# cts198859/deeprl_signal_control

Measured on AMD Instinct MI355X. Metric: env-steps/s (agents x envs x sim-steps/s), large_grid MA2C, higher is better.
Workload: dtype f32; 1 GPU; large_grid 5x5 (25 agents), MA2C LSTM policy (neighbour fingerprint gather), 1024 env instances per GPU; step = 120 control steps (x5 sim-steps) of every instance + 1 A2C update (BPTT, clip, RMSProp); envs_per_gpu=1024, n_step=120, agents=25, parallelism=env-sharded x1, live_vehicles=window mean over the timed region

## Files before the change

deeprl_signal_control_amd/_lib.py:

```python
import ctypes as C
import os

import numpy as np

HERE = os.path.dirname(os.path.abspath(__file__))
LIB_PATH = os.environ.get('TSC_LIB') or os.path.join(HERE, 'libtsc.so')

_fp = C.POINTER(C.c_float)
_ip = C.POINTER(C.c_int32)
_bp = C.POINTER(C.c_uint8)


class TscScenario(C.Structure):
    _fields_ = [
        ('n_lane', C.c_int32), ('n_route', C.c_int32), ('n_agent', C.c_int32), ('n_flow', C.c_int32),
        ('k_max', C.c_int32), ('p_max', C.c_int32), ('l_max', C.c_int32), ('s_max', C.c_int32),
        ('nbr_max', C.c_int32),
        ('lane_len', _fp), ('lane_vmax', _fp), ('lane_det_start', _fp),
        ('lane_node', _ip), ('lane_up', _ip),
        ('mv_next', _ip), ('mv_link', _ip), ('mv_yield', _ip), ('mv_prio', _ip), ('mv_zip', _ip), ('route_entry', _ip), ('flows', _ip),
        ('agent_lanes', _ip), ('agent_nlane', _ip), ('agent_nlink', _ip), ('agent_nphase', _ip),
        ('green_tab', _bp), ('yellow_tab', _bp),
        ('nbr', _ip), ('obs_kind', _ip), ('obs_src', _ip),
        ('control_interval_sec', C.c_int32), ('yellow_interval_sec', C.c_int32),
        ('episode_length_sec', C.c_int32), ('teleport_sec', C.c_int32),
        ('queue_cap', C.c_int32), ('objective', C.c_int32), ('agent_kind', C.c_int32),
        ('realnet_scale', C.c_int32),
        ('coop_gamma', C.c_double), ('norm_wave', C.c_double), ('norm_wait', C.c_double),
        ('clip_wave', C.c_double), ('clip_wait', C.c_double), ('coef_wait', C.c_double),
        ('lane_origin', _fp),
        ('n_stream', C.c_int32), ('k_choice', C.c_int32),
        ('stream_entry', _ip), ('stream_origin', _fp), ('stream_limit', _fp), ('stream_mode', _ip), ('stream_choice', _ip),
        ('n_interval', C.c_int32), ('choice_interval_sec', C.c_int32),
        ('lane_sib', _ip),
    ]


_LIB = None

SYMBOLS = ['tsc_last_error', 'tsc_version', 'tsc_profile_enable', 'tsc_profile_select', 'tsc_profile_reset', 'tsc_profile_read',
           'tsc_profile_name', 'tsc_env_create', 'tsc_env_destroy', 'tsc_env_set_stream', 'tsc_env_set_resident_instances',
           'tsc_env_reset', 'tsc_env_set_stream_routes', 'tsc_env_set_demand', 'tsc_env_demand', 'tsc_env_set_greedy', 'tsc_env_greedy_actions', 'tsc_env_set_pressure', 'tsc_env_pressure_actions', 'tsc_env_set_actuated', 'tsc_env_actuated_actions', 'tsc_env_actuated_state', 'tsc_env_set_reward_pressure', 'tsc_env_fixed_time_actions', 'tsc_env_set_fingerprint', 'tsc_env_bind_fingerprint', 'tsc_env_reward_sum', 'tsc_env_step', 'tsc_env_step_plan', 'tsc_env_get_state',
           'tsc_env_live_vehicles', 'tsc_env_vehicle_counts', 'tsc_env_set_block_order', 'tsc_env_counters', 'tsc_env_debug_clock', 'tsc_env_live_sum', 'tsc_env_record', 'tsc_env_read_record', 'tsc_env_read_trips', 'tsc_env_trace', 'tsc_env_read_trace', 'tsc_env_lane_data', 'tsc_env_read_lane_data', 'tsc_env_set_car_following', 'tsc_env_car_following',
           'tsc_model_create', 'tsc_model_destroy', 'tsc_model_set_stream', 'tsc_model_layout', 'tsc_model_path', 'tsc_model_plan',
           'tsc_model_set_params', 'tsc_model_reset_opt_state', 'tsc_model_debug_read', 'tsc_model_get_params', 'tsc_model_get_opt_state', 'tsc_model_set_opt_state',
           'tsc_model_reset', 'tsc_model_forward', 'tsc_model_forward_sample', 'tsc_model_sample', 'tsc_model_add_transition',
           'tsc_model_rollout_slot', 'tsc_model_compute_grads', 'tsc_model_grad_buffer', 'tsc_model_apply_grads', 'tsc_model_compute_grads_ppo', 'tsc_model_apply_grads_ex', 'tsc_model_ppo_stats', 'tsc_model_get_returns', 'tsc_model_debug_clock',
           'tsc_gemm_grouped_f32',
           'tsc_iql_create', 'tsc_iql_destroy', 'tsc_iql_set_stream', 'tsc_iql_layout', 'tsc_iql_set_params', 'tsc_iql_get_params',
           'tsc_iql_get_opt_state', 'tsc_iql_set_opt_state', 'tsc_iql_forward', 'tsc_iql_add_transition', 'tsc_iql_replay_size',
           'tsc_iql_compute_grads', 'tsc_iql_compute_grads_at', 'tsc_iql_grad_buffer', 'tsc_iql_apply_grads', 'tsc_iql_debug_batch', 'tsc_iql_path', 'tsc_iql_debug_clock',
           'tsc_iql_set_target', 'tsc_iql_sync_target', 'tsc_iql_set_target_params', 'tsc_iql_get_target_params', 'tsc_iql_debug_targets',
           'tsc_iql_set_per', 'tsc_iql_set_per_beta', 'tsc_iql_get_priorities', 'tsc_iql_set_priorities', 'tsc_iql_debug_per',
           'tsc_iql_set_dueling', 'tsc_iql_get_dueling',
           'tsc_iql_set_return_steps', 'tsc_iql_get_return_steps', 'tsc_iql_debug_nstep']


def lib():
    global _LIB
    if _LIB is not None:
        return _LIB
    if not os.path.exists(LIB_PATH):
        raise RuntimeError('deeprl_signal_control_amd: %s not built -- run `python -c "import __graft_entry__ as g; '
                           'g.build()"` (hipcc, gfx950). There is no CPU fallback.' % LIB_PATH)
    import torch
    L = C.CDLL(LIB_PATH)
    vp = C.c_void_p
    L.tsc_last_error.restype = C.c_char_p
    L.tsc_profile_name.restype = C.c_char_p
    L.tsc_profile_name.argtypes = [C.c_int32]
    L.tsc_profile_enable.argtypes = [C.c_int32]
# ... 146 lines not shown
```

deeprl_signal_control_amd/agents.py:

```python
import ctypes as C
import os

import numpy as np
import torch

from . import _lib

A2C_DEFAULTS = dict(rmsp_alpha=0.99, rmsp_epsilon=1e-5, max_grad_norm=40.0, gamma=0.99, lr_init=5e-4,
                    lr_decay='constant', entropy_coef_init=0.01, entropy_coef_min=0.01,
                    entropy_decay='constant', entropy_ratio=0.5, value_coef=0.5, num_fw=128, num_ft=32,
                    num_lstm=64, num_fp=64, batch_size=120, reward_norm=2000.0, reward_clip=2.0,
                    lr_min=0.0)
PPO_DEFAULTS = dict(algo='a2c', ppo_epochs=4, ppo_clip=0.2, gae_lambda=0.95)


def check_algo_config(cfg):
    algo = str(cfg['algo']).strip().lower()
    if algo not in ('a2c', 'ppo'):
        raise ValueError("MODEL_CONFIG algo = %r: expected 'a2c' or 'ppo'" % (cfg['algo'],))
    epochs, clip, lam = cfg['ppo_epochs'], cfg['ppo_clip'], cfg['gae_lambda']
    if not isinstance(epochs, int) or isinstance(epochs, bool) or epochs < 1:
        raise ValueError('MODEL_CONFIG ppo_epochs = %r: expected an integer >= 1' % (epochs,))
    if not (isinstance(clip, (int, float)) and clip > 0):
        raise ValueError('MODEL_CONFIG ppo_clip = %r: expected a number > 0' % (clip,))
# ... 170 lines not shown
def allreduce_grads_(flat_grad, group=None):
    dist = torch.distributed
    if not (dist.is_available() and dist.is_initialized()):
        return 1.0
    world = dist.get_world_size(group)
    dist.all_reduce(flat_grad, op=dist.ReduceOp.SUM, group=group)
    return 1.0 / world


def shard_seeds(seed0, n_env, rank):
    return [seed0 + rank * n_env + e for e in range(n_env)]


def _setup_lib(L):
    if getattr(L, '_model_ready', False):
        return
    vp = C.c_void_p
    L.tsc_model_create.argtypes = [C.POINTER(TscModelCfg), C.c_int32, C.c_int32, C.POINTER(vp)]
    L.tsc_model_destroy.argtypes = [vp]
    L.tsc_model_set_stream.argtypes = [vp, vp]
    L.tsc_model_layout.argtypes = [vp, C.POINTER(C.c_int64)]
    L.tsc_model_path.argtypes = [vp, C.POINTER(C.c_int32)]
    L.tsc_model_plan.argtypes = [vp, C.POINTER(C.c_int32)]
    for f in ('tsc_model_set_params', 'tsc_model_get_params', 'tsc_model_get_opt_state', 'tsc_model_set_opt_state'):
        getattr(L, f).argtypes = [vp, vp]
    L.tsc_model_reset_opt_state.argtypes = [vp]
    L.tsc_model_debug_read.argtypes = [vp, C.c_int32, C.c_int32, C.c_int64, C.c_int64, vp]
    L.tsc_model_reset.argtypes = [vp]
    L.tsc_model_forward.argtypes = [vp, vp, vp, vp, vp, C.c_int32]
    L.tsc_model_sample.argtypes = [vp, vp, vp, C.c_uint64, C.c_uint64]
    L.tsc_model_forward_sample.argtypes = [vp, vp, vp, vp, vp, vp, C.c_uint64, C.c_uint64, C.c_int32]
    L.tsc_model_add_transition.argtypes = [vp, C.c_int32, vp, vp, vp, vp, vp, vp]
    L.tsc_model_rollout_slot.argtypes = [vp, C.c_int32, C.POINTER(vp)]
    L.tsc_model_compute_grads.argtypes = [vp, vp, C.c_double]
    L.tsc_model_grad_buffer.argtypes = [vp, C.POINTER(vp), C.POINTER(C.c_int64)]
    L.tsc_model_apply_grads.argtypes = [vp, C.c_double, C.c_double, vp]
    L.tsc_model_compute_grads_ppo.argtypes = [vp, vp, C.c_double, C.c_double, C.c_double, C.c_int32]
    L.tsc_model_apply_grads_ex.argtypes = [vp, C.c_double, C.c_double, vp, C.c_int32]
    L.tsc_model_ppo_stats.argtypes = [vp, vp]
    L.tsc_model_get_returns.argtypes = [vp, vp, vp]
    L.tsc_model_debug_clock.argtypes = [vp, C.c_int32, vp, C.c_int32]
    L.tsc_gemm_grouped_f32.argtypes = [C.c_int32] * 6 + [vp, C.c_int64, C.c_int32, vp, C.c_int64, C.c_int32,
                                                        vp, C.c_int64, C.c_int32, vp, vp, vp, vp, vp, C.c_int64, vp, C.c_int64, vp]
    L._model_ready = True


class VecA2C:

    def __init__(self, n_s_ls, n_a_ls, n_w_ls, n_f_ls, n_env, s_max, a_max, model_config=None,
                 total_step=0, device=0, seed=None, name='ma2c', process_group=None, policy='lstm', replica=0):
        if not torch.cuda.is_available():
            raise RuntimeError('VecA2C needs a GPU (MI355X); there is no CPU fallback')
        cfg = coerce_config(model_config, {**A2C_DEFAULTS, **PPO_DEFAULTS})
        self.algo, self.ppo_epochs, self.ppo_clip, self.gae_lambda = check_algo_config(cfg)
        self.n_epoch = self.ppo_epochs if self.algo == 'ppo' else 1
        self.cfg, self.name = cfg, name
        self.policy = policy
        self.n_agent, self.E = len(n_s_ls), int(n_env)
        self.n_s_ls, self.n_a_ls, self.n_w_ls, self.n_f_ls = map(list, (n_s_ls, n_a_ls, n_w_ls, n_f_ls))
        if name != 'ma2c':
            self.n_f_ls = [0] * self.n_agent
        self.n_wave_ls = [s - w - f for s, w, f in zip(self.n_s_ls, self.n_w_ls, self.n_f_ls)]
        self.n_step = int(cfg['batch_size'])
        self.s_max, self.a_max = int(s_max), int(a_max)
        self.device = torch.device('cuda', device) if not isinstance(device, torch.device) else device
        self.pg = process_group
# ... 10 lines not shown
        n_ft = int(cfg['num_ft']) if max(self.n_w_ls) > 0 else 0
        mc = TscModelCfg(self.n_agent, self.s_max, self.a_max, *[a.ctypes.data_as(ip) for a in self._arrs],
                         int(cfg['num_fw']), n_ft, n_fp, int(cfg['num_lstm']), self.n_step, float(cfg['gamma']),
                         float(cfg['reward_norm']), float(cfg['reward_clip']), float(cfg['value_coef']),
                         float(cfg['max_grad_norm']), float(cfg['rmsp_alpha']), float(cfg['rmsp_epsilon']),
                         1 if policy == 'fc' else 0)
        self.n_fc = (int(cfg['num_fw']), n_fp, n_ft)
        h = C.c_void_p()
        _lib.check(L.tsc_model_create(C.byref(mc), self.E, self.device.index or 0, C.byref(h)))
        self._h = h
        lay = (C.c_int64 * 12)()
        _lib.check(L.tsc_model_layout(h, lay))
        (self.G, self.stride, self.H, self.Lh, self.oW1, self.ob1, self.oWx, self.oWh, self.obl, self.oWo,
         self.obo, self.out_pad) = [int(x) for x in lay]
        self.layout = ParamLayout(self.n_wave_ls, self.n_w_ls, self.n_f_ls, self.n_a_ls, self.s_max, self.n_fc,
                                  self.Lh, self.out_pad, policy)
        assert self.layout.as_tuple() == tuple(int(x) for x in lay), 'host / device parameter layouts disagree'
        path = (C.c_int32 * 2)()
        _lib.check(L.tsc_model_path(h, path))
        self.fc_path = (int(path[0]), int(path[1]))
        plan = (C.c_int32 * 6)()
        _lib.check(L.tsc_model_plan(h, plan))
        self.plan = tuple(int(x) for x in plan)
        with torch.cuda.device(self.device):
            self.stream = torch.cuda.current_stream(self.device)
            _lib.check(L.tsc_model_set_stream(h, C.c_void_p(self.stream.cuda_stream)))
            d = self.device
            self.pi = torch.zeros(self.E, self.n_agent, self.a_max, dtype=torch.float32, device=d)
            self.v = torch.zeros(self.E, self.n_agent, dtype=torch.float32, device=d)
            self.v_boot = torch.zeros(self.E, self.n_agent, dtype=torch.float32, device=d)
            self.action = torch.zeros(self.E, self.n_agent, dtype=torch.int32, device=d)
            self._false = torch.zeros(self.E, dtype=torch.uint8, device=d)
        gp, cnt = C.c_void_p(), C.c_int64()
        _lib.check(L.tsc_model_grad_buffer(h, C.byref(gp), C.byref(cnt)))
        self._grad_ptr, self.n_param = gp.value, int(cnt.value)
        self.cur_t = 0
        self.sample_step = 0
        dist = torch.distributed
        self.rank = dist.get_rank(process_group) if dist.is_available() and dist.is_initialized() else 0
        self.world = dist.get_world_size(process_group) if dist.is_available() and dist.is_initialized() else 1
        self.base_seed, self.replica = (0 if seed is None else int(seed)), int(replica)
        self.sample_seed = replica_sample_seed(self.base_seed, self.rank, replica)
        self.init_params(seed)
        self.sync_replicas()

    def _init_scheduler(self):
# ... 305 lines not shown
```

deeprl_signal_control_amd/csrc/tsc_env.hip:

```cpp
#include "tsc_common.h"
#include "../../include/tsc.h"

#include <algorithm>
#include <cmath>
#include <cstdlib>
#include <vector>

namespace {

constexpr float kLen = 5.0f, kS0 = 2.0f ,
                kAcc = 5.0f, kDec = 10.0f, kTHead = 1.0f;
constexpr float kICab = 0.070710678f , kHalt = 0.1f, kYieldT = 3.0f, kYieldD = 10.0f;
constexpr int kCap = TSC_LANE_CAP, kMaxCross = TSC_MAX_CROSS, kMaxUp = TSC_MAX_UP;
#ifndef TSC_LANE_MAJOR
#define TSC_LANE_MAJOR 1
#endif
__host__ __device__ __forceinline__ int vslot(int i, int q, int NLP) { return TSC_LANE_MAJOR ? q * kCap + i : i * NLP + q; }

constexpr int kMaxEntry = 8;
__host__ __device__ __forceinline__ int mv_tl(int w) { const int t = w & 0xFFF; return t == 0xFFF ? -1 : t == 0xFFE ? -2 : t; }
__host__ __device__ __forceinline__ int mv_k(int w) { const int k = (w >> 12) & 0x3F; return k == 63 ? -1 : k; }
__host__ __device__ __forceinline__ int mv_yield(int w) { const int y = (w >> 18) & 0xFFF; return y == 0xFFF ? -1 : y; }
__host__ __device__ __forceinline__ bool mv_prio(int w) { return (w >> 30) & 1; }

// ... 1715 lines not shown
}

int tsc_profile_read(int32_t kernel_id, double *total_ms, int64_t *count) {
    if (kernel_id < 0 || kernel_id >= tsc::KID_COUNT || !total_ms || !count) return tsc::fail("tsc_profile_read: bad arguments");
    if (prof_fold()) return 1;
    const tsc::ProfState &p = tsc::prof();
    const long long timed = p.count[kernel_id], all = p.seq[kernel_id];
    *total_ms = timed ? p.total_ms[kernel_id] / (double)timed * (double)all : 0.0;
    *count = all;
    return 0;
}

const char *tsc_profile_name(int32_t id) {
    static const char *names[] = {"env_step", "fc_gemm", "zx_gemm", "lstm_fwd", "head_fwd", "sample", "add_transition",
                                  "returns", "head_bwd", "lstm_bwd", "dwo_gemm", "dwh_gemm", "dwx_gemm", "dx1_gemm",
                                  "dw1_gemm", "grad_norm", "rmsprop", "transpose_wx", "fingerprint", "policy_fwd_fused",
                                  "iql_act", "iql_grad", "iql_reduce", "iql_sample", "iql_add", "iql_adam", "iql_target",
                                  "iql_per_sample", "iql_per_update", "iql_per_add", "iql_nstep", "pressure", "pressure_reward", "actuated", "demand",
                                  "gae", "head_bwd_ppo"};
    static_assert(sizeof(names) / sizeof(names[0]) == tsc::KID_COUNT, "one name per kernel id");
    return (id >= 0 && id < tsc::KID_COUNT) ? names[id] : "";
}

int tsc_version(void) { return 120; }

int tsc_env_create(const tsc_scenario *sc, int32_t n_env, int32_t device, tsc_env **out) {
    if (!sc || !out || n_env <= 0) return tsc::fail("tsc_env_create: bad arguments");
    if (sc->n_lane < 1 || sc->n_route < 1 || sc->n_agent < 1)
        return tsc::fail("tsc_env_create: %d lanes, %d routes, %d agents: a scenario needs at least one of each", sc->n_lane, sc->n_route, sc->n_agent);
    if (sc->n_lane > 1024) return tsc::fail("tsc_env_create: n_lane %d > 1024 unsupported (one thread per live lane): split the network", sc->n_lane);
    if (sc->n_route > 254) return tsc::fail("tsc_env_create: n_route %d > 254 unsupported (route ids are bytes on the device): let disjoint parts of the network share route indices", sc->n_route);
    TSC_HIP(hipSetDevice(device));
    tsc_env *h = new tsc_env();
    tsc::CreateGuard<tsc_env, tsc_env_destroy> guard(h);
    h->device = device;
    h->stream = nullptr;
    EnvDev &P = h->P;
    P.NL = sc->n_lane; P.NLP = (sc->n_lane + 63) / 64 * 64; P.NR = sc->n_route; P.A = sc->n_agent;
    P.KMAX = sc->k_max; P.PMAX = sc->p_max; P.LMAX = sc->l_max; P.SMAX = sc->s_max;
    P.NBR = sc->nbr_max; P.E = n_env;
    P.ctrl = sc->control_interval_sec; P.yellow = sc->yellow_interval_sec; P.episode = sc->episode_length_sec;
    P.teleport = sc->teleport_sec; P.queue_cap = sc->queue_cap; P.objective = sc->objective;
    P.agent_kind = sc->agent_kind; P.realnet_scale = sc->realnet_scale;
    P.coop_gamma = sc->coop_gamma; P.norm_wave = sc->norm_wave; P.norm_wait = sc->norm_wait;
    P.clip_wave = sc->clip_wave; P.clip_wait = sc->clip_wait; P.coef_wait = sc->coef_wait;

    const int NL = P.NL, NR = P.NR, A = P.A;
// ... 1069 lines not shown
```

deeprl_signal_control_amd/csrc/tsc_model.hip:

```cpp
#include "tsc_common.h"
#include "tsc_gemm.h"
#include "../../include/tsc.h"

#include <cstdlib>
#include <type_traits>
#include <vector>

namespace {

using tsc::f32x16;
using tsc::f32x4;
using tsc::GemmArgs;

constexpr int kOut = 8;
constexpr int kL = 64;
constexpr int kG4 = 4 * kL;

struct Layout {
    int G, A, SMAX, AMAX, H;
    int NZ, fc;
    long long stride, oW1, ob1, oWx, oWh, obl, oWo, obo;
};

__device__ __forceinline__ float sigmoidf_(float x) {
// ... 1657 lines not shown
        USTAMP(2, c);
        __builtin_amdgcn_sched_barrier(0);
        if (!lead) stage();
#pragma unroll
        for (int ks = 0; ks < KC / kDwK; ++ks) bcur[ks] = bnxt[ks];
        USTAMP(3, c);
    };
    if (R > 0) {
        for (int c = 0; c < 4; ++c) { fetch_a(Clamp{}, c); commit_a(c); }
        fetch_a(Clamp{}, 4); fetch_b(Clamp{}, bcur, 0);
        __syncthreads();
        long long c = 0;
        for (; KC * (c + 9) <= R; c += 4) {
            sub(Plain{}, c); sub(Plain{}, c + 1); sub(Plain{}, c + 2); sub(Plain{}, c + 3);
            __syncthreads();
            USTAMP(4, c + 3);
        }
        for (; KC * c < R; ++c) {
            sub(Clamp{}, c);
            if ((c & 3) == 3) __syncthreads();
        }
    }
#undef USTAMP
    float *w = ws + ((long long)sp * G + g) * dwxh_ws_floats(H);
#pragma unroll
    for (int t = 0; t < NT; ++t)
#pragma unroll
        for (int r = 0; r < 16; ++r) {
            const int row = 32 * t + (r & 3) + 8 * (r >> 2) + 4 * kh;
            w[(long long)row * kG4 + col0 + li] = acc[t][r];
        }
    bsum += __shfl_xor(bsum, 32, 64);
    if (kh == 0) w[(long long)NT * 32 * kG4 + col0 + li] = bsum;
}

__global__ void dwxh_reduce_kernel(const float *__restrict__ ws, int G, int S, long long per, float *__restrict__ grads,
                                   long long stride, long long off) {
    const long long i = (long long)blockIdx.x * blockDim.x + threadIdx.x;
    if (i >= per * G) return;
    const long long g = i / per, j = i % per;
    float acc = 0.f;
    for (int s = 0; s < S; ++s) acc += ws[((long long)s * G + g) * per + j];
    grads[g * stride + off + j] = acc;
}

constexpr int kD1Ld = 260;
// ... 400 lines not shown
            const int16_t *q = rr + ((g >> 1) * SMAX + f) * 2;
            if (n < q[0] || n >= q[1]) acc = 0.f;
            grads[g * stride + oW1 + j] = acc;
        } else {
            grads[g * stride + ob1 + n] = acc;
        }
    } else {
        const long long jj = j - out1;
        for (int s = 0; s < S; ++s) acc += ws[((long long)s * G + g) * per + w1_ws_floats(H) + jj];
        grads[g * stride + oWx + jj] = acc;
    }
}

namespace {

constexpr size_t kLdsMax = 160 * 1024;

template <int... W> struct Widths {};
using FusedWidths = Widths<128, 160, 192, 224>;
template <int... W, class F> bool with_width(Widths<W...>, int H, F &&f) { return ((H == W && (f(std::integral_constant<int, W>{}), true)) || ...); }
template <class F> bool with_fused_width(int H, F &&f) { return with_width(FusedWidths{}, H, f); }

template <int... W> constexpr bool fused_kernels_fit(Widths<W...>) {
    return ((policy_fwd_fc_mfma_lds(W) <= kLdsMax && dwxh_lds<(W + kL) / 32>() <= kLdsMax && fc_bwd_lds(W) <= kLdsMax) && ...);
}
static_assert(fused_kernels_fit(FusedWidths{}) && dx1w1_lds() <= kLdsMax && lstm_fwd_lds() <= kLdsMax && lstm_bwd2_lds() <= kLdsMax,
              "a kernel's dynamic LDS exceeds the workgroup's");

enum class Fwd : int8_t {
    Dense,
    Tile,
    Ws,
    FcThread,
    FcMfma
};
inline bool fills_cache(Fwd f) { return f == Fwd::Tile || f == Fwd::Ws || f == Fwd::FcMfma; }

struct Plan {
    Fwd fwd;
    bool dwxh;
    bool dx1w1;
    bool fc_bwd;
    int s_fwd;
    int s_upd;
};

}

struct tsc_model {
    Layout lay;
    Plan plan;
    int E, T, device;
    double gamma, rnorm, rclip, vcoef, max_norm, alpha, eps;
    hipStream_t stream;
    tsc::DeviceBufs bufs;
    int *n_act;
    int16_t *rowrange;
    int *wgmap; unsigned fwd_wgs;
    int dbg_tid;
    int *ftmask;
    int *krange;
    float *params, *grads, *ms, *WxT;
    float *Wg;
// ... 125 lines not shown
    TSC_HIP(m->bufs.alloc(&m->norm_part, A * kNormParts, true));
    m->logp_old = nullptr; m->ppo_ready = 0;
    m->ws_floats = (size_t)48 << 20; m->wsc_floats = (size_t)1 << 20;
    TSC_HIP(m->bufs.alloc(&m->ws, m->ws_floats, true)); TSC_HIP(m->bufs.alloc(&m->wsc, m->wsc_floats, true));
    m->dbg = nullptr;
    m->cached_next = 0;
    m->inplace = 0;

    const auto env_int = [](const char *name, int unset) { const char *ev = getenv(name); return ev ? atoi(ev) : unset; };
    const char *fwd_ws = getenv("TSC_FWD_WS");
    const bool unfused_dx = env_int("TSC_UNFUSED_DX", 0) != 0;
    m->dbg_tid = env_int("TSC_DBG_THREAD", 0);
    Plan &P = m->plan;
    P.s_upd = 256 / (int)G;
    if (P.s_upd < 1) P.s_upd = 1;
    P.s_fwd = P.s_upd < (E + 31) / 32 ? P.s_upd : (int)((E + 31) / 32);
    const bool wide = with_fused_width(L.H, [](auto) {}), narrow_obs = L.SMAX <= 64;
    const auto ws_fits = [&](long long per_split) { return (size_t)(P.s_upd * G * per_split) <= m->ws_floats; };
    if (!L.fc) {
        const bool tile = L.H % 32 == 0 && narrow_obs && policy_fwd_fused_lds(L.H) <= kLdsMax;
        P.fwd = !tile ? Fwd::Dense
              : wide && policy_fwd_ws_lds(L.H, L.SMAX) <= kLdsMax && !(fwd_ws && fwd_ws[0] == '0') ? Fwd::Ws : Fwd::Tile;
        P.dwxh = wide && !env_int("TSC_UNFUSED_DW", 0) && ws_fits(dwxh_ws_floats(L.H));
        P.dx1w1 = wide && narrow_obs && !unfused_dx && ws_fits(w1_ws_floats(L.H));
    } else {
        P.fwd = wide && narrow_obs && env_int("TSC_FC_MFMA", 1) ? Fwd::FcMfma
              : L.H % 16 == 0 && narrow_obs && fc_thread_lds(L.H) <= kLdsMax ? Fwd::FcThread : Fwd::Dense;
        P.fc_bwd = wide && narrow_obs && !unfused_dx && ws_fits(fc_bwd_ws_floats(L.H));
    }
    m->fwd_wgs = (unsigned)(G * P.s_fwd);
    if (P.fwd == Fwd::Ws && env_int("TSC_FWD_XCD", 1) && P.s_fwd > 1 && P.s_fwd < 256) {
        const int S = P.s_fwd, cap = (L.G * S + 7) / 8;
        std::vector<int> tab((size_t)8 * cap, -1), used(8, 0);
        for (int gg = 0; gg < L.G; ++gg) {
            int left = S, spn = 0;
            while (left > 0) {
                int x = 0;
                for (int k = 1; k < 8; ++k) if (cap - used[k] > cap - used[x]) x = k;
                const int take = left < cap - used[x] ? left : cap - used[x];
                for (int q = 0; q < take; ++q) tab[(size_t)(used[x] + q) * 8 + x] = (gg << 8) | (spn + q);
                used[x] += take; spn += take; left -= take;
            }
        }
        TSC_HIP(m->bufs.upload(&m->wgmap, tab.data(), tab.size()));
        m->fwd_wgs = (unsigned)tab.size();
    }
    hipError_t attr = hipSuccess;
    const auto allow_lds = [&attr](const void *k) {
        if (attr == hipSuccess) attr = hipFuncSetAttribute(k, hipFuncAttributeMaxDynamicSharedMemorySize, (int)kLdsMax);
    };
    allow_lds((const void *)lstm_bwd2_kernel);
    allow_lds((const void *)lstm_fwd_kernel<true>);
    allow_lds((const void *)lstm_fwd_kernel<false>);
    if (P.fwd == Fwd::Tile) allow_lds((const void *)policy_fwd_fused_kernel);
    if (P.fwd == Fwd::FcThread) allow_lds((const void *)policy_fwd_fc_kernel);
    with_fused_width(L.H, [&](auto w) {
        constexpr int H = decltype(w)::value;
        if (P.fwd == Fwd::Ws) allow_lds((const void *)policy_fwd_ws_kernel<(H + kL) / 2>);
        if (P.fwd == Fwd::FcMfma) allow_lds((const void *)policy_fwd_fc_mfma_kernel<H / 32>);
        if (P.dwxh) allow_lds((const void *)dwxh_kernel<(H + kL) / 32>);
        if (P.dx1w1) allow_lds((const void *)dx1w1_kernel2<H / 16>);
        if (P.fc_bwd) allow_lds((const void *)fc_bwd_kernel<H / 16>);
    });
    TSC_HIP(attr);
    hipLaunchKernelGGL(fill_kernel, dim3((unsigned)((m->nparam + 255) / 256)), dim3(256), 0, 0, m->ms, m->nparam, 1.0f);
    TSC_HIP(hipDeviceSynchronize());
    *out = guard.release();
    return 0;
}

int tsc_model_destroy(tsc_model *m) {
    if (!m) return 0;
    (void)hipSetDevice(m->device);
    delete m;
    return 0;
}

int tsc_model_set_stream(tsc_model *m, void *s) {
    if (!m) return tsc::fail("null handle");
    m->stream = (hipStream_t)s;
    return 0;
}

// ... 35 lines not shown
}
int tsc_model_set_opt_state(tsc_model *m, const float *h) {
    if (!m || !h) return tsc::fail("tsc_model_set_opt_state: bad arguments");
    TSC_HIP(hipStreamSynchronize(m->stream));
    TSC_HIP(hipMemcpy(m->ms, h, sizeof(float) * m->nparam, hipMemcpyHostToDevice));
    return 0;
}

int tsc_model_reset(tsc_model *m) {
    if (!m) return tsc::fail("null handle");
    const size_t b = sizeof(float) * (size_t)m->lay.G * m->E * 2 * kL;
    TSC_HIP(hipMemsetAsync(m->state_fw, 0, b, m->stream));
    TSC_HIP(hipMemsetAsync(m->state_bw, 0, b, m->stream));
    m->ppo_ready = 0;
    return 0;
}

int tsc_model_path(tsc_model *m, int32_t out[2]) {
    if (!m || !out) return tsc::fail("tsc_model_path: bad arguments");
    const bool fc = m->lay.fc != 0;
    const Fwd f = m->plan.fwd;
    out[0] = !fc ? -1 : f == Fwd::FcMfma ? 2 : f == Fwd::FcThread ? 1 : 0;
    out[1] = !fc ? -1 : m->plan.fc_bwd ? 1 : 0;
    return 0;
}

int tsc_model_plan(tsc_model *m, int32_t out[6]) {
    if (!m || !out) return tsc::fail("tsc_model_plan: bad arguments");
    const Plan &P = m->plan;
    const int32_t v[6] = {(int32_t)P.fwd, P.dwxh, P.dx1w1, P.fc_bwd, P.s_fwd, P.s_upd};
    for (int i = 0; i < 6; ++i) out[i] = v[i];
    return 0;
}

static int model_forward(tsc_model *m, const float *obs, const uint8_t *done, float *pi, float *v, int32_t advance,
                         int32_t *action, uint64_t seed, uint64_t step, int32_t tslot) {
    if (!m || !obs || !done || !pi || !v) return tsc::fail("tsc_model_forward: bad arguments");
    const Layout &L = m->lay;
    const Plan &P = m->plan;
    const int E = m->E;
    if (advance) {
        if (tslot == 0) m->cached_next = 0;
        if (fills_cache(P.fwd) && tslot >= 0 && tslot == m->cached_next && tslot < m->T) m->cached_next = tslot + 1;
        else { m->cached_next = -1; tslot = -1; }
    } else {
        tslot = -1;
// ... 135 lines not shown
    }
    {
        tsc::ProfScope ps(tsc::KID_DWO_GEMM, m->stream);
        const int tot = L.A * 2 * (kL * kOut + kOut);
        hipLaunchKernelGGL(head_bwd2_reduce_kernel, dim3((tot + 255) / 256), dim3(256), 0, st, m->ws, L.A, S, m->grads, L);
    }
    return hipGetLastError() == hipSuccess ? 0 : 1;
}

int tsc_model_rollout_slot(tsc_model *m, int32_t t, void *ptrs[6]) {
    if (!m || !ptrs || t < 0 || t > m->T) return tsc::fail("tsc_model_rollout_slot: slot %d outside [0,%d]", t, m ? m->T : 0);
    const Layout &L = m->lay;
    const long long E = m->E, A = L.A, no = E * A * L.SMAX;
    const bool in = t < m->T;
    ptrs[0] = m->r_obs + t * no;
    ptrs[1] = in ? (void *)(m->r_act + t * E * A) : nullptr;
    ptrs[2] = in ? (void *)(m->r_val + t * E * A) : nullptr;
    ptrs[3] = in ? (void *)(m->r_rew + t * E * A) : nullptr;
    ptrs[4] = m->r_done + t * E;
    ptrs[5] = in ? (void *)(m->r_done + (t + 1) * E) : nullptr;
    return 0;
}

static void launch_dwxh(tsc_model *m, long long N) {
    const Layout &L = m->lay;
    const int G = L.G, S = m->plan.s_upd;
    const long long per = dwxh_ws_floats(L.H);
    {
        tsc::ProfScope ps(tsc::KID_DWX_GEMM, m->stream);
        with_fused_width(L.H, [&](auto w) {
            constexpr int NT = (decltype(w)::value + kL) / 32;
            hipLaunchKernelGGL(dwxh_kernel<NT>, dim3((unsigned)(S * G)), dim3(512), dwxh_lds<NT>(), m->stream, m->X1, m->Hp, m->Z, N, G, S,
                               split_rows(N, S, kDwK), m->ws, m->dbg);
        });
    }
    tsc::ProfScope ps(tsc::KID_DWH_GEMM, m->stream);
    hipLaunchKernelGGL(dwxh_reduce_kernel, dim3((unsigned)((per * G + 255) / 256)), dim3(256), 0, m->stream, m->ws, G, S, per, m->grads,
                       L.stride, L.oWx);
}

static void launch_w1(tsc_model *m, long long N) {
    const Layout &L = m->lay;
    const int G = L.G, S = m->plan.s_upd;
    const long long rps = split_rows(N, S, kW1Chunk), perF = L.fc ? fc2_ws_floats(L.H) : 0;
    {
        tsc::ProfScope ps(tsc::KID_DX1_GEMM, m->stream);
        with_fused_width(L.H, [&](auto w) {
            constexpr int H = decltype(w)::value;
            if (L.fc)
                hipLaunchKernelGGL(fc_bwd_kernel<H / 16>, dim3((unsigned)(S * G)), dim3(512), fc_bwd_lds(H), m->stream, m->dHh, m->X1, m->WxT,
                                   m->r_obs, N, G, S, rps, L.A, L.SMAX, m->ws, m->ftmask);
            else
                hipLaunchKernelGGL(dx1w1_kernel2<H / 16>, dim3((unsigned)(S * G)), dim3(512), dx1w1_lds(), m->stream, m->Z, m->X1, m->WxT,
                                   m->r_obs, N, G, S, rps, L.A, L.SMAX, m->ws, m->ftmask, m->dbg);
        });
    }
    tsc::ProfScope ps(tsc::KID_DW1_GEMM, m->stream);
    const long long tot = ((long long)(L.SMAX + 1) * L.H + perF) * G;
    hipLaunchKernelGGL(w1_reduce_kernel, dim3((unsigned)((tot + 255) / 256)), dim3(256), 0, m->stream, m->ws, G, S, L.H, L.SMAX, perF,
                       m->rowrange, m->grads, L.stride, L.oW1, L.ob1, L.oWx);
}
// ... 202 lines not shown
        case 5: base = m->dHh; w = kL; break;
        default: return tsc::fail("tsc_model_debug_read: unknown buffer %d", what);
    }
    if (m->lay.fc && (what == 1 || what == 3 || what == 4)) return tsc::fail("tsc_model_debug_read: buffer %d is LSTM-only", what);
    TSC_HIP(hipStreamSynchronize(m->stream));
    TSC_HIP(hipMemcpy(out_host, base + ((long long)g * N + row0) * w, sizeof(float) * (size_t)(nrows * w), hipMemcpyDeviceToHost));
    return 0;
}

int tsc_gemm_grouped_f32(int32_t form, int32_t epi, int32_t groups, int32_t M, int32_t N, int32_t K, const float *A,
                         int64_t sA, int32_t lda, const float *B, int64_t sB, int32_t ldb, float *C, int64_t sC,
                         int32_t ldc, const float *bias, const float *aux, const int16_t *rowrange, float *colsum,
                         float *splitk_ws, int64_t ws_floats, float *splitk_wsc, int64_t wsc_floats, void *hip_stream) {
    GemmArgs a;
    a.A = A; a.B = B; a.C = C; a.bias = bias; a.aux = aux; a.rr = rowrange; a.colsum = colsum;
    a.sA = sA; a.sB = sB; a.sC = sC; a.sBias = N; a.sAux = (long long)M * ldc; a.sRR = M; a.sColsum = N;
    a.lda = lda; a.ldb = ldb; a.ldc = ldc; a.ldaux = ldc; a.M = M; a.N = N; a.K = K; a.gdivA = 1;
    tsc::plan_splitk(a, groups, form != 0 ? splitk_ws : nullptr, splitk_wsc, (size_t)ws_floats, (size_t)wsc_floats);
    tsc::launch_gemm_dyn(form != 0, epi, a, groups, (hipStream_t)hip_stream);
    TSC_HIP(hipGetLastError());
    return 0;
}

}
```

include/tsc.h:

```cpp
#ifndef TSC_H_
#define TSC_H_

#include <stddef.h>
#include <stdint.h>

#ifdef __cplusplus
extern "C" {
#endif

#define TSC_MAX_UP     4
#define TSC_MAX_CROSS  4
#define TSC_LANE_CAP   28

enum { TSC_AGENT_GREEDY = 0, TSC_AGENT_GLOBAL = 1 , TSC_AGENT_MA2C = 2 };
enum { TSC_OBJ_QUEUE = 0, TSC_OBJ_WAIT = 1, TSC_OBJ_HYBRID = 2 };
enum { TSC_CF_IDM = 0, TSC_CF_KRAUSS = 1 };
enum { TSC_PRESSURE_COUNT = 0, TSC_PRESSURE_QUEUE = 1 };

typedef struct tsc_scenario {
    int32_t n_lane, n_route, n_agent, n_flow;
    int32_t k_max;
    int32_t p_max;
    int32_t l_max;
    int32_t s_max;
// ... 104 lines not shown


typedef struct tsc_model_cfg {
    int32_t n_agent;
    int32_t s_max, a_max;
    const int32_t *n_wave;
    const int32_t *n_wait;
    const int32_t *n_fp;
    const int32_t *n_act;
    int32_t n_fc_wave, n_fc_wait, n_fc_fp, n_lstm;
    int32_t n_step;
    double gamma, reward_norm, reward_clip, value_coef, max_grad_norm, rmsp_alpha, rmsp_epsilon;
    int32_t policy_kind;
} tsc_model_cfg;

typedef struct tsc_model tsc_model;

int tsc_model_create(const tsc_model_cfg *cfg, int32_t n_env, int32_t device, tsc_model **out);
int tsc_model_destroy(tsc_model *m);
int tsc_model_set_stream(tsc_model *m, void *hip_stream);
int tsc_model_layout(tsc_model *m, int64_t out[12]);
int tsc_model_path(tsc_model *m, int32_t out[2]);
int tsc_model_plan(tsc_model *m, int32_t out[6]);
int tsc_model_set_params(tsc_model *m, const float *params_host);
int tsc_model_reset_opt_state(tsc_model *m);
int tsc_model_get_params(tsc_model *m, float *params_host);
int tsc_model_get_opt_state(tsc_model *m, float *ms_host);
int tsc_model_set_opt_state(tsc_model *m, const float *ms_host);

int tsc_model_reset(tsc_model *m);

int tsc_model_forward(tsc_model *m, const float *obs_dev, const uint8_t *done_dev, float *pi_dev,
                      float *v_dev, int32_t advance);

int tsc_model_forward_sample(tsc_model *m, const float *obs_dev, const uint8_t *done_dev, float *pi_dev,
                             float *v_dev, int32_t *action_dev, uint64_t seed, uint64_t step, int32_t t_slot);

int tsc_model_sample(tsc_model *m, const float *pi_dev, int32_t *action_dev, uint64_t seed, uint64_t step);

int tsc_model_add_transition(tsc_model *m, int32_t t, const float *obs_dev, const uint8_t *done_pre_dev,
                             const int32_t *action_dev, const double *reward_dev, const float *value_dev,
                             const uint8_t *done_post_dev);

int tsc_model_rollout_slot(tsc_model *m, int32_t t, void *ptrs[6]);

int tsc_model_compute_grads(tsc_model *m, const float *R_boot_dev, double entropy_beta);
// ... 54 lines not shown
int tsc_iql_set_target_params(tsc_iql *h, const float *params_host);
int tsc_iql_get_target_params(tsc_iql *h, float *params_host);
int tsc_iql_debug_targets(tsc_iql *h, float *y_host, int32_t *astar_host);
#define TSC_IQL_PER_MAX_BUFFER 4096
int tsc_iql_set_per(tsc_iql *h, int32_t enable, double alpha, double eps);
int tsc_iql_set_per_beta(tsc_iql *h, double beta);
int tsc_iql_get_priorities(tsc_iql *h, float *prio_host, float *qmax_host);
int tsc_iql_set_priorities(tsc_iql *h, const float *prio_host, const float *qmax_host);
int tsc_iql_debug_per(tsc_iql *h, float *w_host, float *td_host);
int tsc_iql_set_dueling(tsc_iql *h, int32_t enable);
int tsc_iql_get_dueling(tsc_iql *h, int32_t *enabled);
#define TSC_IQL_MAX_RETURN_STEPS 32
int tsc_iql_set_return_steps(tsc_iql *h, int32_t n);
int tsc_iql_get_return_steps(tsc_iql *h, int32_t *n);
int tsc_iql_debug_nstep(tsc_iql *h, int32_t *slot_host, float *ret_host, float *disc_host, int32_t *k_host);
int tsc_iql_debug_clock(tsc_iql *h, int32_t enable, int64_t *stamps_host, int32_t count);

int tsc_gemm_grouped_f32(int32_t form, int32_t epi, int32_t groups, int32_t M, int32_t N, int32_t K,
                         const float *A, int64_t sA, int32_t lda, const float *B, int64_t sB, int32_t ldb,
                         float *C, int64_t sC, int32_t ldc, const float *bias, const float *aux,
                         const int16_t *rowrange, float *colsum, float *splitk_ws, int64_t ws_floats,
                         float *splitk_wsc, int64_t wsc_floats, void *hip_stream);

#ifdef __cplusplus
}
#endif
#endif
```

Baseline: 400.3 million env-steps/s.

## Add split-bf16 MFMA kernel for the LSTM input/hidden weight-gradient GEMM

Adds a dwxh_split_kernel that computes the Wx/Wh weight gradient with bf16 MFMA instructions. Each f32 operand is split into three bf16 parts (hi/mid/lo) and six cross products are accumulated, which approximates f32 accuracy. Operands are staged in swizzled LDS read with transposing ds_read_tr16, using a 4-deep ring buffer and hand-placed scheduling barriers. It is on by default (TSC_DW_SPLIT=1) whenever the fused dwxh path is chosen, and a standalone tsc_dwxh_f32 entry point is added for testing. The cost is six MFMAs per product, more LDS, and slight numeric differences from the previous f32 kernel.

```diff
diff --git a/deeprl_signal_control_amd/_lib.py b/deeprl_signal_control_amd/_lib.py
--- a/deeprl_signal_control_amd/_lib.py
+++ b/deeprl_signal_control_amd/_lib.py
@@ -42,11 +42,11 @@
            'tsc_profile_name', 'tsc_env_create', 'tsc_env_destroy', 'tsc_env_set_stream', 'tsc_env_set_resident_instances',
            'tsc_env_reset', 'tsc_env_set_stream_routes', 'tsc_env_set_demand', 'tsc_env_demand', 'tsc_env_set_greedy', 'tsc_env_greedy_actions', 'tsc_env_set_pressure', 'tsc_env_pressure_actions', 'tsc_env_set_actuated', 'tsc_env_actuated_actions', 'tsc_env_actuated_state', 'tsc_env_set_reward_pressure', 'tsc_env_fixed_time_actions', 'tsc_env_set_fingerprint', 'tsc_env_bind_fingerprint', 'tsc_env_reward_sum', 'tsc_env_step', 'tsc_env_step_plan', 'tsc_env_get_state',
            'tsc_env_live_vehicles', 'tsc_env_vehicle_counts', 'tsc_env_set_block_order', 'tsc_env_counters', 'tsc_env_debug_clock', 'tsc_env_live_sum', 'tsc_env_record', 'tsc_env_read_record', 'tsc_env_read_trips', 'tsc_env_trace', 'tsc_env_read_trace', 'tsc_env_lane_data', 'tsc_env_read_lane_data', 'tsc_env_set_car_following', 'tsc_env_car_following',
-           'tsc_model_create', 'tsc_model_destroy', 'tsc_model_set_stream', 'tsc_model_layout', 'tsc_model_path', 'tsc_model_plan',
+           'tsc_model_create', 'tsc_model_destroy', 'tsc_model_set_stream', 'tsc_model_layout', 'tsc_model_path', 'tsc_model_plan', 'tsc_model_dw_split',
            'tsc_model_set_params', 'tsc_model_reset_opt_state', 'tsc_model_debug_read', 'tsc_model_get_params', 'tsc_model_get_opt_state', 'tsc_model_set_opt_state',
            'tsc_model_reset', 'tsc_model_forward', 'tsc_model_forward_sample', 'tsc_model_sample', 'tsc_model_add_transition',
            'tsc_model_rollout_slot', 'tsc_model_compute_grads', 'tsc_model_grad_buffer', 'tsc_model_apply_grads', 'tsc_model_compute_grads_ppo', 'tsc_model_apply_grads_ex', 'tsc_model_ppo_stats', 'tsc_model_get_returns', 'tsc_model_debug_clock',
-           'tsc_gemm_grouped_f32',
+           'tsc_gemm_grouped_f32', 'tsc_dwxh_f32',
            'tsc_iql_create', 'tsc_iql_destroy', 'tsc_iql_set_stream', 'tsc_iql_layout', 'tsc_iql_set_params', 'tsc_iql_get_params',
            'tsc_iql_get_opt_state', 'tsc_iql_set_opt_state', 'tsc_iql_forward', 'tsc_iql_add_transition', 'tsc_iql_replay_size',
            'tsc_iql_compute_grads', 'tsc_iql_compute_grads_at', 'tsc_iql_grad_buffer', 'tsc_iql_apply_grads', 'tsc_iql_debug_batch', 'tsc_iql_path', 'tsc_iql_debug_clock',
diff --git a/deeprl_signal_control_amd/agents.py b/deeprl_signal_control_amd/agents.py
--- a/deeprl_signal_control_amd/agents.py
+++ b/deeprl_signal_control_amd/agents.py
@@ -216,6 +216,7 @@
     L.tsc_model_layout.argtypes = [vp, C.POINTER(C.c_int64)]
     L.tsc_model_path.argtypes = [vp, C.POINTER(C.c_int32)]
     L.tsc_model_plan.argtypes = [vp, C.POINTER(C.c_int32)]
+    L.tsc_model_dw_split.argtypes = [vp, C.POINTER(C.c_int32)]
     for f in ('tsc_model_set_params', 'tsc_model_get_params', 'tsc_model_get_opt_state', 'tsc_model_set_opt_state'):
         getattr(L, f).argtypes = [vp, vp]
     L.tsc_model_reset_opt_state.argtypes = [vp]
@@ -236,6 +237,7 @@
     L.tsc_model_debug_clock.argtypes = [vp, C.c_int32, vp, C.c_int32]
     L.tsc_gemm_grouped_f32.argtypes = [C.c_int32] * 6 + [vp, C.c_int64, C.c_int32, vp, C.c_int64, C.c_int32,
                                                         vp, C.c_int64, C.c_int32, vp, vp, vp, vp, vp, C.c_int64, vp, C.c_int64, vp]
+    L.tsc_dwxh_f32.argtypes = [C.c_int32, C.c_int64, C.c_int32, C.c_int32, vp, vp, vp, vp, C.c_int32]
     L._model_ready = True
 
 
@@ -292,6 +294,9 @@
         plan = (C.c_int32 * 6)()
         _lib.check(L.tsc_model_plan(h, plan))
         self.plan = tuple(int(x) for x in plan)
+        dws = C.c_int32()
+        _lib.check(L.tsc_model_dw_split(h, C.byref(dws)))
+        self.dw_split = int(dws.value)
         with torch.cuda.device(self.device):
             self.stream = torch.cuda.current_stream(self.device)
             _lib.check(L.tsc_model_set_stream(h, C.c_void_p(self.stream.cuda_stream)))
diff --git a/deeprl_signal_control_amd/csrc/tsc_env.hip b/deeprl_signal_control_amd/csrc/tsc_env.hip
--- a/deeprl_signal_control_amd/csrc/tsc_env.hip
+++ b/deeprl_signal_control_amd/csrc/tsc_env.hip
@@ -1761,7 +1761,7 @@
     return (id >= 0 && id < tsc::KID_COUNT) ? names[id] : "";
 }
 
-int tsc_version(void) { return 120; }
+int tsc_version(void) { return 121; }
 
 int tsc_env_create(const tsc_scenario *sc, int32_t n_env, int32_t device, tsc_env **out) {
     if (!sc || !out || n_env <= 0) return tsc::fail("tsc_env_create: bad arguments");
diff --git a/deeprl_signal_control_amd/csrc/tsc_model.hip b/deeprl_signal_control_amd/csrc/tsc_model.hip
--- a/deeprl_signal_control_amd/csrc/tsc_model.hip
+++ b/deeprl_signal_control_amd/csrc/tsc_model.hip
@@ -1703,6 +1703,200 @@
         }
     }
 #undef USTAMP
+    float *w = ws + ((long long)sp * G + g) * dwxh_ws_floats(H);
+#pragma unroll
+    for (int t = 0; t < NT; ++t)
+#pragma unroll
+        for (int r = 0; r < 16; ++r) {
+            const int row = 32 * t + (r & 3) + 8 * (r >> 2) + 4 * kh;
+            w[(long long)row * kG4 + col0 + li] = acc[t][r];
+        }
+    bsum += __shfl_xor(bsum, 32, 64);
+    if (kh == 0) w[(long long)NT * 32 * kG4 + col0 + li] = bsum;
+}
+
+typedef __bf16 bf16x4 __attribute__((ext_vector_type(4)));
+typedef __bf16 bf16x8 __attribute__((ext_vector_type(8)));
+typedef short s16x4 __attribute__((ext_vector_type(4)));
+typedef short s16x8 __attribute__((ext_vector_type(8)));
+typedef s16x4 __attribute__((address_space(3))) *lds_s16x4_p;
+
+constexpr int kDsKi = 32;
+template <int NT> constexpr size_t dwxh_split_plane() { return sizeof(__bf16) * kDwKc * NT * 32; }
+template <int NT> constexpr size_t dwxh_split_lds() { return 3 * dwxh_split_plane<NT>() * (2 * kDsKi / kDwKc); }
+__device__ __forceinline__ constexpr unsigned dwxh_split_off(int NT, int rr, int f) {
+    return ((rr >> 3) * NT + (f >> 5)) * 512 + 64 * (rr & 7) + 16 * (((f >> 3) & 3) ^ ((rr >> 2) & 3)) + 2 * (f & 7);
+}
+
+template <int NT>
+__global__ void __launch_bounds__(512, 1)
+dwxh_split_kernel(const float *__restrict__ X1, const float *__restrict__ Hp, const float *__restrict__ dZ, long long N, int G,
+                  int S, long long rows_per_split, float *__restrict__ ws) {
+    constexpr int HT = NT - 2, H = 32 * HT, KC = kDwKc;
+    constexpr int XQ = H / 4, NX = KC * XQ;
+    constexpr unsigned PL = (unsigned)dwxh_split_plane<NT>(), SUB = 3 * PL;
+    static_assert(NX >= 512 && NX <= 1024 && NX % 64 == 0 && KC * (kL / 4) == 256, "staging slots");
+    static_assert(2 * PL + (NT - 1) * 512 < 65536, "a fragment read's immediate offset");
+    extern __shared__ __attribute__((aligned(16))) char smem_raw[];
+    const int g = blockIdx.x % G, sp = blockIdx.x / G;
+    const int tid = threadIdx.x, lane = tid & 63, wave = __builtin_amdgcn_readfirstlane(tid >> 6), li = lane & 31, kh = lane >> 5;
+    const int col0 = 32 * wave;
+    const auto uniform = [](long long v) {
+        const unsigned lo = __builtin_amdgcn_readfirstlane((unsigned)v), hi = __builtin_amdgcn_readfirstlane((unsigned)((unsigned long long)v >> 32));
+        return (long long)(((unsigned long long)hi << 32) | lo);
+    };
+    const long long n0 = uniform((long long)sp * rows_per_split);
+    const long long n1 = uniform(n0 + rows_per_split > N ? N : n0 + rows_per_split);
+    const int R = __builtin_amdgcn_readfirstlane((int)(n1 - n0));
+    const float *x1 = X1 + (long long)g * N * H, *hp = Hp + (long long)g * N * kL;
+    const float *dz = dZ + (long long)g * N * kG4;
+    f32x16 acc[NT];
+#pragma unroll
+    for (int t = 0; t < NT; ++t)
+#pragma unroll
+        for (int r = 0; r < 16; ++r) acc[t][r] = 0.f;
+    float bsum = 0.f;
+    const bool has1 = wave < (NX - 512) / 64, has2 = wave >= 4;
+    struct Slots { int r0, c0, r1, c1, r2, c2; };
+    auto slots = [&](int t) {
+        const int i1 = has1 ? t + 512 : t, i2 = t & 255;
+        return Slots{t / XQ, 4 * (t % XQ), i1 / XQ, 4 * (i1 % XQ), i2 >> 4, 4 * (i2 & 15)};
+    };
+    const Slots sl = slots(tid);
+    const unsigned o0 = sl.r0 * H + sl.c0, o1 = sl.r1 * H + sl.c1, o2 = sl.r2 * kL + sl.c2;
+    const unsigned l0 = dwxh_split_off(NT, sl.r0, sl.c0), l1 = dwxh_split_off(NT, sl.r1, sl.c1),
+                   l2 = dwxh_split_off(NT, sl.r2, H + sl.c2);
+    const int rq = (lane >> 2) & 3, rp = lane & 3, rc = 2 * ((lane >> 4) & 1) + (rp >> 1);
+    const unsigned rb0 = kh * NT * 512 + 64 * rq + 16 * (rc ^ (2 * kh)) + 8 * (rp & 1),
+                   rb1 = kh * NT * 512 + 64 * (4 + rq) + 16 * (rc ^ (2 * kh + 1)) + 8 * (rp & 1);
+    const unsigned zb = 8 * kh * kG4 + col0 + li;
+    f32x4 g0, g1, g2;
+    bf16x8 b1, b2, b3;
+    float bnxt[8];
+    using Clamp = std::true_type;
+    using Plain = std::false_type;
+    auto fetch_a = [&](auto cl, long long c) {
+        if constexpr (decltype(cl)::value) {
+            int t = tid;
+            asm volatile("" : "+v"(t));
+            const Slots q = slots(t);
+            auto rowc = [&](long long r) { return r < n1 ? r : n1 - 1; };
+            const long long b = n0 + KC * c;
+            g0 = *reinterpret_cast<const f32x4 *>(x1 + rowc(b + q.r0) * H + q.c0);
+            if (has1) g1 = *reinterpret_cast<const f32x4 *>(x1 + rowc(b + q.r1) * H + q.c1);
+            if (has2) g2 = *reinterpret_cast<const f32x4 *>(hp + rowc(b + q.r2) * kL + q.c2);
+        } else {
+            const gfloat_p xs = uniform_ptr(x1 + (n0 + KC * c) * H), hs = uniform_ptr(hp + (n0 + KC * c) * kL);
+            g0 = *(gfloat4_p)(xs + o0);
+            if (has1) g1 = *(gfloat4_p)(xs + o1);
+            if (has2) g2 = *(gfloat4_p)(hs + o2);
+        }
+    };
+    auto put = [&](char *d, const f32x4 &v) {
+        bf16x4 p1, p2, p3;
+#pragma unroll
+        for (int e = 0; e < 4; ++e) {
+            p1[e] = (__bf16)v[e];
+            const float r1 = v[e] - (float)p1[e];
+            p2[e] = (__bf16)r1;
+            p3[e] = (__bf16)(r1 - (float)p2[e]);
+        }
+        *reinterpret_cast<bf16x4 *>(d) = p1;
+        *reinterpret_cast<bf16x4 *>(d + PL) = p2;
+        *reinterpret_cast<bf16x4 *>(d + 2 * PL) = p3;
+    };
+    auto commit_a = [&](long long c) {
+        char *d = smem_raw + (unsigned)(c & 3) * SUB;
+        put(d + l0, g0);
+        if (has1) put(d + l1, g1);
+        if (has2) put(d + l2, g2);
+    };
+    auto fetch_b = [&](auto cl, long long c) {
+        if constexpr (decltype(cl)::value) {
+            int t = tid;
+            asm volatile("" : "+v"(t));
+            const long long row0 = n0 + KC * c + 8 * ((t >> 5) & 1);
+            const float *zc = dz + col0 + (t & 31);
+#pragma unroll
+            for (int j = 0; j < 8; ++j) {
+                const long long row = row0 + j;
+                const float z = zc[(row < n1 ? row : n1 - 1) * kG4];
+                bnxt[j] = row < n1 ? z : 0.f;
+            }
+        } else {
+            const gfloat_p zs = uniform_ptr(dz + (n0 + KC * c) * kG4);
+#pragma unroll
+            for (int j = 0; j < 8; ++j) bnxt[j] = (zs + j * kG4)[zb];
+        }
+    };
+    auto split_b = [&]() {
+#pragma unroll
+        for (int j = 0; j < 8; ++j) {
+            bsum += bnxt[j];
+            b1[j] = (__bf16)bnxt[j];
+            const float r1 = bnxt[j] - (float)b1[j];
+            b2[j] = (__bf16)r1;
+            b3[j] = (__bf16)(r1 - (float)b2[j]);
+        }
+    };
+    const bool lead = wave < 4;
+    auto sub = [&](auto cl, long long c) {
+        auto stage = [&]() { commit_a(c + 2); fetch_a(cl, c + 3); };
+        fetch_b(cl, c + 1);
+        if (lead) stage();
+        const char *a = smem_raw + (unsigned)(c & 3) * SUB;
+        const lds_s16x4_p a0 = (lds_s16x4_p)(a + rb0), a1 = (lds_s16x4_p)(a + rb1);
+        __builtin_amdgcn_sched_barrier(0);
+        auto frag = [&](int t, int p) {
+            const s16x4 lo = __builtin_amdgcn_ds_read_tr16_b64_v4i16(a0 + (p * PL + t * 512) / 8);
+            const s16x4 hi = __builtin_amdgcn_ds_read_tr16_b64_v4i16(a1 + (p * PL + t * 512) / 8);
+            return __builtin_bit_cast(bf16x8, (s16x8)__builtin_shufflevector(lo, hi, 0, 1, 2, 3, 4, 5, 6, 7));
+        };
+        bf16x8 p1[2], p2, p3;
+        p3 = frag(0, 2); p1[0] = frag(0, 0); p2 = frag(0, 1);
+        __builtin_amdgcn_sched_group_barrier(0x100, 6, 0);
+#pragma unroll
+        for (int t = 0; t < NT; ++t) {
+            const bool more = t + 1 < NT;
+            const bf16x8 c1 = p1[t & 1];
+            acc[t] = __builtin_amdgcn_mfma_f32_32x32x16_bf16(p3, b1, acc[t], 0, 0, 0);
+            if (more) p3 = frag(t + 1, 2);
+            acc[t] = __builtin_amdgcn_mfma_f32_32x32x16_bf16(c1, b3, acc[t], 0, 0, 0);
+            if (more) p1[(t + 1) & 1] = frag(t + 1, 0);
+            acc[t] = __builtin_amdgcn_mfma_f32_32x32x16_bf16(p2, b2, acc[t], 0, 0, 0);
+            acc[t] = __builtin_amdgcn_mfma_f32_32x32x16_bf16(p2, b1, acc[t], 0, 0, 0);
+            if (more) p2 = frag(t + 1, 1);
+            acc[t] = __builtin_amdgcn_mfma_f32_32x32x16_bf16(c1, b2, acc[t], 0, 0, 0);
+            acc[t] = __builtin_amdgcn_mfma_f32_32x32x16_bf16(c1, b1, acc[t], 0, 0, 0);
+            if (more) {
+                __builtin_amdgcn_sched_group_barrier(0x008, 1, 0);
+                __builtin_amdgcn_sched_group_barrier(0x100, 2, 0);
+                __builtin_amdgcn_sched_group_barrier(0x008, 1, 0);
+                __builtin_amdgcn_sched_group_barrier(0x100, 2, 0);
+                __builtin_amdgcn_sched_group_barrier(0x008, 2, 0);
+                __builtin_amdgcn_sched_group_barrier(0x100, 2, 0);
+                __builtin_amdgcn_sched_group_barrier(0x008, 2, 0);
+            }
+        }
+        __builtin_amdgcn_sched_barrier(0);
+        if (!lead) stage();
+        split_b();
+    };
+    if (R > 0) {
+        for (int c = 0; c < 2; ++c) { fetch_a(Clamp{}, c); commit_a(c); }
+        fetch_a(Clamp{}, 2); fetch_b(Clamp{}, 0);
+        split_b();
+        __syncthreads();
+        int c = 0;
+        for (; KC * (c + 5) <= R; c += 2) {
+            sub(Plain{}, c); sub(Plain{}, c + 1);
+            __syncthreads();
+        }
+        for (; KC * c < R; ++c) {
+            sub(Clamp{}, c);
+            if (c & 1) __syncthreads();
+        }
+    }
     float *w = ws + ((long long)sp * G + g) * dwxh_ws_floats(H);
 #pragma unroll
     for (int t = 0; t < NT; ++t)
@@ -2149,7 +2343,8 @@
 template <class F> bool with_fused_width(int H, F &&f) { return with_width(FusedWidths{}, H, f); }
 
 template <int... W> constexpr bool fused_kernels_fit(Widths<W...>) {
-    return ((policy_fwd_fc_mfma_lds(W) <= kLdsMax && dwxh_lds<(W + kL) / 32>() <= kLdsMax && fc_bwd_lds(W) <= kLdsMax) && ...);
+    return ((policy_fwd_fc_mfma_lds(W) <= kLdsMax && dwxh_lds<(W + kL) / 32>() <= kLdsMax && dwxh_split_lds<(W + kL) / 32>() <= kLdsMax &&
+             fc_bwd_lds(W) <= kLdsMax) && ...);
 }
 static_assert(fused_kernels_fit(FusedWidths{}) && dx1w1_lds() <= kLdsMax && lstm_fwd_lds() <= kLdsMax && lstm_bwd2_lds() <= kLdsMax,
               "a kernel's dynamic LDS exceeds the workgroup's");
@@ -2166,6 +2361,7 @@
 struct Plan {
     Fwd fwd;
     bool dwxh;
+    bool dw_split;
     bool dx1w1;
     bool fc_bwd;
     int s_fwd;
@@ -2337,6 +2533,7 @@
         P.fwd = !tile ? Fwd::Dense
               : wide && policy_fwd_ws_lds(L.H, L.SMAX) <= kLdsMax && !(fwd_ws && fwd_ws[0] == '0') ? Fwd::Ws : Fwd::Tile;
         P.dwxh = wide && !env_int("TSC_UNFUSED_DW", 0) && ws_fits(dwxh_ws_floats(L.H));
+        P.dw_split = P.dwxh && env_int("TSC_DW_SPLIT", 1) != 0;
         P.dx1w1 = wide && narrow_obs && !unfused_dx && ws_fits(w1_ws_floats(L.H));
     } else {
         P.fwd = wide && narrow_obs && env_int("TSC_FC_MFMA", 1) ? Fwd::FcMfma
@@ -2373,7 +2570,7 @@
         constexpr int H = decltype(w)::value;
         if (P.fwd == Fwd::Ws) allow_lds((const void *)policy_fwd_ws_kernel<(H + kL) / 2>);
         if (P.fwd == Fwd::FcMfma) allow_lds((const void *)policy_fwd_fc_mfma_kernel<H / 32>);
-        if (P.dwxh) allow_lds((const void *)dwxh_kernel<(H + kL) / 32>);
+        if (P.dwxh) allow_lds(P.dw_split ? (const void *)dwxh_split_kernel<(H + kL) / 32> : (const void *)dwxh_kernel<(H + kL) / 32>);
         if (P.dx1w1) allow_lds((const void *)dx1w1_kernel2<H / 16>);
         if (P.fc_bwd) allow_lds((const void *)fc_bwd_kernel<H / 16>);
     });
@@ -2455,6 +2652,12 @@
     const Fwd f = m->plan.fwd;
     out[0] = !fc ? -1 : f == Fwd::FcMfma ? 2 : f == Fwd::FcThread ? 1 : 0;
     out[1] = !fc ? -1 : m->plan.fc_bwd ? 1 : 0;
+    return 0;
+}
+
+int tsc_model_dw_split(tsc_model *m, int32_t *out) {
+    if (!m || !out) return tsc::fail("tsc_model_dw_split: bad arguments");
+    *out = m->plan.dw_split;
     return 0;
 }
 
@@ -2636,21 +2839,31 @@
     return 0;
 }
 
+static void launch_dwxh_pass(int H, bool split, const float *X1, const float *Hp, const float *dZ, long long N, int G, int S, float *ws,
+                             long long *dbg, hipStream_t st) {
+    with_fused_width(H, [&](auto w) {
+        constexpr int NT = (decltype(w)::value + kL) / 32;
+        if (split)
+            hipLaunchKernelGGL(dwxh_split_kernel<NT>, dim3((unsigned)(S * G)), dim3(512), dwxh_split_lds<NT>(), st, X1, Hp, dZ, N, G, S,
+                               split_rows(N, S, kDwK), ws);
+        else
+            hipLaunchKernelGGL(dwxh_kernel<NT>, dim3((unsigned)(S * G)), dim3(512), dwxh_lds<NT>(), st, X1, Hp, dZ, N, G, S,
+                               split_rows(N, S, kDwK), ws, dbg);
+    });
+}
+static void launch_dwxh_reduce(int H, const float *ws, int G, int S, float *grads, long long stride, long long off, hipStream_t st) {
+    const long long per = dwxh_ws_floats(H);
+    hipLaunchKernelGGL(dwxh_reduce_kernel, dim3((unsigned)((per * G + 255) / 256)), dim3(256), 0, st, ws, G, S, per, grads, stride, off);
+}
 static void launch_dwxh(tsc_model *m, long long N) {
     const Layout &L = m->lay;
     const int G = L.G, S = m->plan.s_upd;
-    const long long per = dwxh_ws_floats(L.H);
     {
         tsc::ProfScope ps(tsc::KID_DWX_GEMM, m->stream);
-        with_fused_width(L.H, [&](auto w) {
-            constexpr int NT = (decltype(w)::value + kL) / 32;
-            hipLaunchKernelGGL(dwxh_kernel<NT>, dim3((unsigned)(S * G)), dim3(512), dwxh_lds<NT>(), m->stream, m->X1, m->Hp, m->Z, N, G, S,
-                               split_rows(N, S, kDwK), m->ws, m->dbg);
-        });
+        launch_dwxh_pass(L.H, m->plan.dw_split, m->X1, m->Hp, m->Z, N, G, S, m->ws, m->dbg, m->stream);
     }
     tsc::ProfScope ps(tsc::KID_DWH_GEMM, m->stream);
-    hipLaunchKernelGGL(dwxh_reduce_kernel, dim3((unsigned)((per * G + 255) / 256)), dim3(256), 0, m->stream, m->ws, G, S, per, m->grads,
-                       L.stride, L.oWx);
+    launch_dwxh_reduce(L.H, m->ws, G, S, m->grads, L.stride, L.oWx, m->stream);
 }
 
 static void launch_w1(tsc_model *m, long long N) {
@@ -2899,4 +3112,24 @@
     return 0;
 }
 
-}
+int tsc_dwxh_f32(int32_t H, int64_t N, int32_t G, int32_t S, const float *X1, const float *Hp, const float *dZ, float *out, int32_t split) {
+    if (!X1 || !Hp || !dZ || !out || N < 1 || G < 1 || S < 1) return tsc::fail("tsc_dwxh_f32: bad arguments");
+    if (!with_fused_width(H, [](auto) {})) return tsc::fail("tsc_dwxh_f32: no kernel for H = %d", H);
+    hipError_t attr = hipSuccess;
+    with_fused_width(H, [&](auto w) {
+        constexpr int NT = (decltype(w)::value + kL) / 32;
+        attr = hipFuncSetAttribute(split ? (const void *)dwxh_split_kernel<NT> : (const void *)dwxh_kernel<NT>,
+                                   hipFuncAttributeMaxDynamicSharedMemorySize, (int)kLdsMax);
+    });
+    TSC_HIP(attr);
+    tsc::DeviceBufs bufs;
+    float *ws = nullptr;
+    TSC_HIP(bufs.alloc(&ws, (size_t)S * G * dwxh_ws_floats(H), false));
+    launch_dwxh_pass(H, split != 0, X1, Hp, dZ, N, G, S, ws, nullptr, nullptr);
+    launch_dwxh_reduce(H, ws, G, S, out, dwxh_ws_floats(H), 0, nullptr);
+    TSC_HIP(hipGetLastError());
+    TSC_HIP(hipDeviceSynchronize());
+    return 0;
+}
+
+}
diff --git a/include/tsc.h b/include/tsc.h
--- a/include/tsc.h
+++ b/include/tsc.h
@@ -150,6 +150,7 @@
 int tsc_model_layout(tsc_model *m, int64_t out[12]);
 int tsc_model_path(tsc_model *m, int32_t out[2]);
 int tsc_model_plan(tsc_model *m, int32_t out[6]);
+int tsc_model_dw_split(tsc_model *m, int32_t *out);
 int tsc_model_set_params(tsc_model *m, const float *params_host);
 int tsc_model_reset_opt_state(tsc_model *m);
 int tsc_model_get_params(tsc_model *m, float *params_host);
@@ -250,6 +251,9 @@
                          const int16_t *rowrange, float *colsum, float *splitk_ws, int64_t ws_floats,
                          float *splitk_wsc, int64_t wsc_floats, void *hip_stream);
 
+int tsc_dwxh_f32(int32_t H, int64_t N, int32_t G, int32_t S, const float *X1, const float *Hp, const float *dZ, float *out,
+                 int32_t split);
+
 #ifdef __cplusplus
 }
 #endif
```

After: 419.9 million env-steps/s (median of 6 runs). 1.05x the previous value.
